# blindopen/TSM-Det-Pointcloud-

Measured on AMD Instinct MI355X. Metric: point-cloud frames/sec (fwd+bwd), higher is better.
Workload: dtype f32; 1 GPU; BASELINE configs[1]: KITTI-shaped synthetic, 20000 pts / 16000 active voxels per frame, full SECOND detector (VoxelBackBone8x) fwd+bwd+AdamW step; batch_per_gpu=4, global_batch=4, parallelism=dp1, voxelize_on_gpu=True

## Files before the change

tsm-det-pointcloud-_amd/csrc/conv_wgrad.hip:

```cpp
#include "spx_common.h"

#ifdef SPX_WG_DIAG
__device__ unsigned long long* g_wg_diag = nullptr;
extern "C" int spx_diag_set(unsigned long long* p) { return (int)hipMemcpyToSymbol(HIP_SYMBOL(g_wg_diag), &p, sizeof(p)); }
#define DIAG_T() __builtin_amdgcn_s_memtime()
#endif

namespace {

typedef float f32x4 __attribute__((ext_vector_type(4)));

#ifndef SPX_SB
#define SPX_SB __builtin_amdgcn_sched_barrier(0)
#endif
constexpr int kGroups = 4;
#ifndef SPX_WG_BURST
#define SPX_WG_BURST 4
#endif
constexpr int kBurst = SPX_WG_BURST;

static inline int wgrad_splits(int64_t n, int cin, int cout, int kvol) {
  int64_t s = n / (64 * kGroups);
  constexpr int slab_mb = 32;
  int64_t by_slab = (int64_t(slab_mb) << 20) / ((int64_t)kvol * cin * cout * 4);
  if (s > by_slab) s = by_slab;
  constexpr int max_blocks = 2048;
  int64_t by_blocks = max_blocks / kvol;
  if (by_blocks < 8) by_blocks = 8;
  if (s > by_blocks) s = by_blocks;
  if (s < 1) s = 1;
  return (int)s;
}

__device__ __forceinline__ void wgrad_plan(const int32_t* __restrict__ cnt, int K, int J, int lane, int& sk, int& start,
                                           int& mycnt) {
  const uint32_t cval = lane < K ? (uint32_t)cnt[lane] : 0u;
  mycnt = (int)cval;
  uint64_t total = cval;
#pragma unroll
  for (int o = 32; o > 0; o >>= 1) total += __shfl_xor(total, o);
  int sh = 0;
  while ((total >> sh) >= (1u << 19)) ++sh;
  const uint32_t tot_s = (uint32_t)(total >> sh);
  sk = 0;
  if (lane < K) sk = tot_s > 0 ? 1 + (int)(((uint32_t)(J - K) * (cval >> sh)) / tot_s) : J / K;
  int incl = sk;
#pragma unroll
  for (int o = 1; o < 64; o <<= 1) {
    int t = __shfl_up(incl, o);
    if (lane >= o) incl += t;
  }
  start = incl - sk;
}

constexpr int kCntUnroll = 4;
__global__ __launch_bounds__(1024) void k_wgrad_count(const int32_t* __restrict__ pair, int64_t ld, int64_t n,
                                                      const int64_t* d_n, int K, int G, int32_t* __restrict__ cnt64,
                                                      int32_t* __restrict__ cnt8) {
  __shared__ int32_t part[16];
  const int x = blockIdx.x, k = blockIdx.y;
  const int lane = threadIdx.x & 63, w = threadIdx.x >> 6;
  const int64_t nlive = spx_live_n(d_n, n);
  const int64_t n8 = ((nlive + 7) / 8 + 63) / 64 * 64;
  const int64_t g0 = x * (n8 / 64);
  int64_t g1 = g0 + n8 / 64;
  const int64_t glive = (nlive + 63) / 64;
  if (g1 > glive) g1 = glive;
  const int32_t* prow = pair + (int64_t)k * ld;
  int total = 0;
  for (int64_t g = g0 + w * kCntUnroll; g < g1; g += 16 * kCntUnroll) {
    int32_t id[kCntUnroll];
#pragma unroll
    for (int u = 0; u < kCntUnroll; ++u) {
      const int64_t row = 64 * (g + u) + lane;
      id[u] = (g + u < g1 && row < nlive) ? prow[row] : -1;
    }
#pragma unroll
    for (int u = 0; u < kCntUnroll; ++u) {
      const int c = __popcll(__ballot(id[u] >= 0));
      if (lane == 0 && g + u < g1) cnt64[(size_t)k * G + g + u] = c;
      total += c;
    }
  }
  if (lane == 0) part[w] = total;
  __syncthreads();
  if (threadIdx.x == 0) {
    int t = 0;
#pragma unroll
    for (int i = 0; i < 16; ++i) t += part[i];
    cnt8[x * 32 + k] = t;
  }
}

template <int W>
__device__ __forceinline__ void load_vec(const float* __restrict__ p, float (&v)[W]) {
  if constexpr (W == 1) {
    v[0] = p[0];
  } else if constexpr (W == 2) {
    float2 t = *reinterpret_cast<const float2*>(p);
    v[0] = t.x, v[1] = t.y;
  } else {
#pragma unroll
    for (int i = 0; i < W; i += 4) {
      float4 t = *reinterpret_cast<const float4*>(p + i);
      v[i] = t.x, v[i + 1] = t.y, v[i + 2] = t.z, v[i + 3] = t.w;
    }
  }
}

template <int W>
__device__ __forceinline__ void store_vec(float* __restrict__ p, const float (&v)[W]) {
  if constexpr (W == 1) {
    p[0] = v[0];
  } else if constexpr (W == 2) {
    *reinterpret_cast<float2*>(p) = make_float2(v[0], v[1]);
  } else {
#pragma unroll
    for (int i = 0; i < W; i += 4) *reinterpret_cast<float4*>(p + i) = make_float4(v[i], v[i + 1], v[i + 2], v[i + 3]);
  }
}

template <int MI, int NJ, bool EXACT, bool FULL>
__device__ __forceinline__ void wgrad_fetch(const float* __restrict__ in, int cin, const float* __restrict__ dout,
                                            int cout, const int32_t* q_src, const int32_t* q_dst, int p, int npairs,
                                            int c, float (&a)[MI], float (&b)[NJ]) {
  const bool has = FULL || (p < npairs);
  const int32_t sid = has ? q_src[p] : 0;
  const int32_t did = has ? q_dst[p] : 0;
  if (EXACT && FULL) {
    load_vec<MI>(in + (size_t)sid * cin + MI * c, a);
    load_vec<NJ>(dout + (size_t)did * cout + NJ * c, b);
  } else {
#pragma unroll
    for (int mi = 0; mi < MI; ++mi) {
      int ci = MI * c + mi;
      a[mi] = (has && ci < cin) ? in[(size_t)sid * cin + ci] : 0.f;
    }
#pragma unroll
    for (int nj = 0; nj < NJ; ++nj) {
      int co = NJ * c + nj;
      b[nj] = (has && co < cout) ? dout[(size_t)did * cout + co] : 0.f;
    }
  }
}

template <int MI, int NJ>
__device__ __forceinline__ void wgrad_mfma_step(f32x4 (&acc)[MI][NJ], const float (&a)[MI], const float (&b)[NJ]) {
#pragma unroll
  for (int mi = 0; mi < MI; ++mi)
#pragma unroll
    for (int nj = 0; nj < NJ; ++nj) acc[mi][nj] = __builtin_amdgcn_mfma_f32_16x16x4f32(a[mi], b[nj], acc[mi][nj], 0, 0, 0);
}

template <int MI, int NJ, bool EXACT>
__global__ __launch_bounds__(64) void k_wgrad_mfma(const float* __restrict__ in, int cin,
                                                   const float* __restrict__ dout, int cout,
                                                   const int32_t* __restrict__ pair, int64_t ld, int64_t n,
                                                   const int64_t* d_n, const int32_t* __restrict__ cnt64,
                                                   const int32_t* __restrict__ cnt8, int G, int J, int K,
                                                   float* __restrict__ slab) {
  __shared__ int32_t q_src[64 * kGroups + 4];
  __shared__ int32_t q_dst[64 * kGroups + 4];
  const int lane = threadIdx.x;
  const int c = lane & 15, q = lane >> 4;
  const int xcd = blockIdx.x & 7, j = blockIdx.x >> 3;
  int sk, start, mycnt;
  wgrad_plan(cnt8 + xcd * 32, K, J, lane, sk, start, mycnt);
  const unsigned long long mine = __ballot(lane < K && j >= start && j < start + sk);
  if (mine == 0) return;
  const int k = __ffsll((long long)mine) - 1;
  const int sub = __builtin_amdgcn_readfirstlane(j - __shfl(start, k));
  const int nsub = __builtin_amdgcn_readfirstlane(__shfl(sk, k));
  const int64_t total = __builtin_amdgcn_readfirstlane(__shfl(mycnt, k));
  const int64_t nlive = spx_live_n(d_n, n);
  const int64_t n8 = ((nlive + 7) / 8 + 63) / 64 * 64;
  const int64_t lo = total * sub / nsub, hi = total * (sub + 1) / nsub;
  const int gx0 = (int)(xcd * (n8 / 64));
  int gx1 = gx0 + (int)(n8 / 64);
  const int glive = (int)((nlive + 63) / 64);
  if (gx1 > glive) gx1 = glive;
  int n_lo = 0, n_hi = 0;
  int64_t run = 0;
  for (int g = gx0; g < gx1; g += 64) {
    const int v = g + lane < gx1 ? cnt64[(size_t)k * G + g + lane] : 0;
    int incl = v;
#pragma unroll
    for (int o = 1; o < 64; o <<= 1) {
      int t = __shfl_up(incl, o);
      if (lane >= o) incl += t;
    }
    const int64_t excl = run + incl - v;
    const bool in = g + lane < gx1;
    n_lo += __popcll(__ballot(in && excl < lo));
    n_hi += __popcll(__ballot(in && excl < hi));
    run += __shfl(incl, 63);
  }
  int64_t r0 = 64 * (int64_t)(gx0 + n_lo);
  int64_t r1 = 64 * (int64_t)(gx0 + n_hi);
  if (r1 > nlive) r1 = nlive;
  if (r0 > r1) r0 = r1;

#ifdef SPX_WG_DIAG
  const unsigned long long d_t0 = DIAG_T(), d_r0 = __builtin_amdgcn_s_memrealtime();
  unsigned long long d_steps = 0, d_loop = 0, d_nsteps = 0;
#endif
  f32x4 acc[MI][NJ];
#pragma unroll
  for (int mi = 0; mi < MI; ++mi)
#pragma unroll
    for (int nj = 0; nj < NJ; ++nj) acc[mi][nj] = f32x4{0.f, 0.f, 0.f, 0.f};

  const int32_t* prow = pair + (int64_t)k * ld;
  int carry = 0;
  int32_t idn[kGroups];
  const int64_t rlast = r1 > r0 ? r1 - 1 : 0;
#pragma unroll
  for (int g = 0; g < kGroups; ++g) {
    int64_t row = r0 + 64 * g + lane;
    idn[g] = prow[row < rlast ? row : rlast];
  }
  for (int64_t base = r0; base < r1; base += 64 * kGroups) {
    int32_t id[kGroups];
#pragma unroll
    for (int g = 0; g < kGroups; ++g) {
      id[g] = base + 64 * g + lane < r1 ? idn[g] : -1;
      int64_t row = base + 64 * (kGroups + g) + lane;
      idn[g] = prow[row < rlast ? row : rlast];
    }
    int nvalid = carry;
#pragma unroll
    for (int g = 0; g < kGroups; ++g) {
      unsigned long long mask = __ballot(id[g] >= 0);
      int rank = nvalid + __builtin_amdgcn_mbcnt_hi((unsigned)(mask >> 32), __builtin_amdgcn_mbcnt_lo((unsigned)mask, 0u));
      if (id[g] >= 0) {
        q_src[rank] = id[g];
        q_dst[rank] = (int32_t)(base + 64 * g + lane);
      }
      nvalid += __popcll(mask);
    }
    const int full = nvalid >> 2;
    carry = nvalid & 3;
    if (full == 0) continue;
    __builtin_amdgcn_wave_barrier();
    const int last = full - 1;
#ifdef SPX_WG_DIAG
    const unsigned long long d_a = DIAG_T();
    d_nsteps += full;
#endif
    for (int st = 0; st < full; st += kBurst) {
      float a[kBurst][MI], b[kBurst][NJ];
#pragma unroll
      for (int g = 0; g < kBurst; ++g) {
        const int sg = st + g < last ? st + g : last;
        wgrad_fetch<MI, NJ, EXACT, true>(in, cin, dout, cout, q_src, q_dst, 4 * sg + q, 4, c, a[g], b[g]);
      }
      asm volatile("" ::: "memory");
      __builtin_amdgcn_sched_barrier(0);
#pragma unroll
      for (int g = 0; g < kBurst; ++g) {
        if (g > 0) {
          const float keep = st + g < full ? 1.f : 0.f;
#pragma unroll
          for (int nj = 0; nj < NJ; ++nj) b[g][nj] *= keep;
        }
        wgrad_mfma_step<MI, NJ>(acc, a[g], b[g]);
      }
    }
#ifdef SPX_WG_DIAG
    d_loop += DIAG_T() - d_a;
#endif
    __builtin_amdgcn_wave_barrier();
    if (carry) {
      int32_t ts = 0, td = 0;
      if (lane < carry) ts = q_src[4 * full + lane], td = q_dst[4 * full + lane];
      __builtin_amdgcn_wave_barrier();
      if (lane < carry) q_src[lane] = ts, q_dst[lane] = td;
    }
    __builtin_amdgcn_wave_barrier();
  }
  int ntail = carry ? 1 : 0;
  ntail = __builtin_amdgcn_readfirstlane(ntail);
  asm volatile("" : "+s"(ntail));
  for (int t = 0; t < ntail; ++t) {
    __builtin_amdgcn_wave_barrier();
    float a0[MI], b0[NJ];
    wgrad_fetch<MI, NJ, EXACT, false>(in, cin, dout, cout, q_src, q_dst, q, carry, c, a0, b0);
    wgrad_mfma_step<MI, NJ>(acc, a0, b0);
  }

#ifdef SPX_WG_DIAG
  if (g_wg_diag && lane == 0) {
    unsigned long long* o = g_wg_diag + (size_t)blockIdx.x * 8;
    const unsigned long long t1 = DIAG_T();
    o[0] = t1 - d_t0;
    o[1] = d_loop;
    o[2] = d_nsteps;
    o[3] = __builtin_amdgcn_s_memrealtime() - d_r0;
    o[4] = k;
    o[5] = d_t0;
    o[6] = t1;
    o[7] = (unsigned long long)(r1 > r0 ? r1 - r0 : 0);
  }
#endif
  float* out = slab + ((size_t)xcd * J + j) * cin * cout;
#pragma unroll
  for (int mi = 0; mi < MI; ++mi)
#pragma unroll
    for (int e = 0; e < 4; ++e) {
      const int ci = MI * (4 * q + e) + mi;
      if (EXACT) {
        float v[NJ];
#pragma unroll
        for (int nj = 0; nj < NJ; ++nj) v[nj] = acc[mi][nj][e];
        store_vec<NJ>(out + (size_t)ci * cout + NJ * c, v);
      } else if (ci < cin) {
#pragma unroll
        for (int nj = 0; nj < NJ; ++nj) {
          int co = NJ * c + nj;
          if (co < cout) out[(size_t)ci * cout + co] = acc[mi][nj][e];
        }
      }
    }
}

constexpr int kRedSlices = 16;
__global__ __launch_bounds__(64 * kRedSlices) void k_wgrad_reduce(const float* __restrict__ slab,
                                                                   const int32_t* __restrict__ cnt8, int J, int K, int cin,
                                                                   int cout, float* __restrict__ dw) {
  __shared__ float part[kRedSlices][64];
  __shared__ int p_off[9][32], p_start[8][32];
  {
    const int w = threadIdx.x >> 6, lane = threadIdx.x & 63;
    if (w < 8) {
      int sk, start, mycnt;
      wgrad_plan(cnt8 + w * 32, K, J, lane, sk, start, mycnt);
      if (lane < 32) p_off[w + 1][lane] = sk, p_start[w][lane] = start;
    }
  }
  __syncthreads();
  if (threadIdx.x < 32) {
    int run = 0;
    for (int x = 0; x < 8; ++x) {
      int v = p_off[x + 1][threadIdx.x];
      p_off[x][threadIdx.x] = run;
      run += v;
    }
    p_off[8][threadIdx.x] = run;
  }
  __syncthreads();
  const int per = cin * cout;
  const int total = K * per;
  const int e = threadIdx.x & 63, sl = threadIdx.x >> 6;
  const int t = blockIdx.x * 64 + e;
  float acc4[4] = {0.f, 0.f, 0.f, 0.f};
  if (t < total) {
    const int k = t / per, el = t - k * per;
    const int len = p_off[8][k];
    int x = 0;
    for (int i = sl; i < len; i += 4 * kRedSlices) {
#pragma unroll
      for (int u = 0; u < 4; ++u) {
        const int ii = i + u * kRedSlices;
        if (ii < len) {
          while (ii >= p_off[x + 1][k]) ++x;
          acc4[u] += slab[((size_t)x * J + p_start[x][k] + (ii - p_off[x][k])) * per + el];
        }
      }
    }
  }
  part[sl][e] = (acc4[0] + acc4[1]) + (acc4[2] + acc4[3]);
  __syncthreads();
  if (sl == 0 && t < total) {
    float v = 0.f;
#pragma unroll
    for (int i = 0; i < kRedSlices; ++i) v += part[i][e];
    int co = t % cout, ci = (t / cout) % cin, k = t / per;
    dw[((size_t)co * K + k) * cin + ci] = v;
  }
}

}

static inline int wgrad_blocks_per_xcd(int64_t n, int cin, int cout, int kvol) {
  int J = (wgrad_splits(n, cin, cout, kvol) * kvol + 7) / 8;
  return J < kvol ? kvol : J;
}

static inline size_t wgrad_slab_bytes(int cin, int cout, int kvol, int64_t n) {
  return spx_align((size_t)8 * wgrad_blocks_per_xcd(n, cin, cout, kvol) * cin * cout * sizeof(float));
}
static inline size_t wgrad_cnt64_bytes(int kvol, int64_t n) {
  return spx_align((size_t)kvol * (size_t)((n + 63) / 64 + 1) * sizeof(int32_t));
}

extern "C" size_t spx_conv_wgrad_ws_bytes(int cin, int cout, int kvol, int64_t n_out) {
  return wgrad_slab_bytes(cin, cout, kvol, n_out) + wgrad_cnt64_bytes(kvol, n_out) + spx_align(8 * 32 * sizeof(int32_t));
}

#define SPX_WG_CASE(A, B)                                                                                          \
  if (MI == A && NJ == B) {                                                                                        \
    if (exact)                                                                                                     \
      hipLaunchKernelGGL((k_wgrad_mfma<A, B, true>), dim3(8 * J), dim3(64), 0, s, in, cin, dout, cout, pair, pair_ld, n_out, \
                         d_n_out, cnt64, cnt8, G, J, kvol, slab);                                                  \
    else                                                                                                           \
      hipLaunchKernelGGL((k_wgrad_mfma<A, B, false>), dim3(8 * J), dim3(64), 0, s, in, cin, dout, cout, pair, pair_ld, n_out, \
                         d_n_out, cnt64, cnt8, G, J, kvol, slab);                                                  \
    launched = true;                                                                                               \
  }

extern "C" size_t spx_conv_wgrad_counts_bytes(int kvol, int64_t n_out) {
  return wgrad_cnt64_bytes(kvol, n_out < 0 ? 0 : n_out) + spx_align(8 * 32 * sizeof(int32_t));
}

extern "C" int spx_conv_wgrad_counts(const int32_t* pair, int64_t pair_ld, int kvol, int64_t n_out, const int64_t* d_n_out,
                                     int32_t* counts, spx_stream_t stream) {
  if (!pair || !counts || kvol <= 0 || kvol > SPX_MAX_KVOL || n_out <= 0 || pair_ld < n_out) return SPX_ERR_INVALID_ARG;
  if (n_out >= (int64_t(1) << 31)) return SPX_ERR_TOO_LARGE;
  const int G = (int)((n_out + 63) / 64 + 1);
  int32_t* cnt8 = reinterpret_cast<int32_t*>(reinterpret_cast<char*>(counts) + wgrad_cnt64_bytes(kvol, n_out));
  hipLaunchKernelGGL(k_wgrad_count, dim3(8, kvol), dim3(1024), 0, spx_s(stream), pair, pair_ld, n_out, d_n_out, kvol, G,
                     counts, cnt8);
  SPX_CHECK_LAUNCH();
  return SPX_OK;
}

extern "C" int spx_conv_wgrad(const float* in, int cin, const float* dout, int cout, int kvol, const int32_t* pair,
                              int64_t pair_ld, int64_t n_out, const int64_t* d_n_out, const int32_t* counts, float* dw,
                              void* ws, size_t ws_bytes, spx_stream_t stream) {
  if (!in || !dout || !pair || !dw || cin <= 0 || cout <= 0 || kvol <= 0 || kvol > SPX_MAX_KVOL || n_out < 0 ||
      pair_ld < n_out)
    return SPX_ERR_INVALID_ARG;
  if (cin > 128 || cout > 128) return SPX_ERR_UNSUPPORTED;
  if (n_out >= (int64_t(1) << 31)) return SPX_ERR_TOO_LARGE;
  if (!ws || ws_bytes < spx_conv_wgrad_ws_bytes(cin, cout, kvol, n_out)) return SPX_ERR_WORKSPACE;
  hipStream_t s = spx_s(stream);
  if (n_out == 0) {
    spx_fill_async(dw, 0, sizeof(float) * (size_t)cout * kvol * cin, s);
    return SPX_OK;
  }
  const int J = wgrad_blocks_per_xcd(n_out, cin, cout, kvol);
  const int G = (int)((n_out + 63) / 64 + 1);
  const int32_t* cnt64 = counts;
  const int32_t* cnt8 = counts ? reinterpret_cast<const int32_t*>(reinterpret_cast<const char*>(counts) + wgrad_cnt64_bytes(kvol, n_out))
                               : nullptr;
  if (!counts) {
    int32_t* c64 = reinterpret_cast<int32_t*>(reinterpret_cast<char*>(ws) + wgrad_slab_bytes(cin, cout, kvol, n_out));
    int32_t* c8 = reinterpret_cast<int32_t*>(reinterpret_cast<char*>(c64) + wgrad_cnt64_bytes(kvol, n_out));
    hipLaunchKernelGGL(k_wgrad_count, dim3(8, kvol), dim3(1024), 0, s, pair, pair_ld, n_out, d_n_out, kvol, G, c64, c8);
    cnt64 = c64;
    cnt8 = c8;
  }
  float* slab = reinterpret_cast<float*>(ws);
  int MI = (cin + 15) / 16, NJ = (cout + 15) / 16;
  if (MI == 3) MI = 4;
  if (MI > 4) MI = 8;
  if (NJ == 3) NJ = 4;
  if (NJ > 4) NJ = 8;
  bool launched = false;
  const bool exact = cin == 16 * MI && cout == 16 * NJ;
  SPX_WG_CASE(1, 1)
  SPX_WG_CASE(1, 2)
  SPX_WG_CASE(1, 4)
  SPX_WG_CASE(1, 8)
  SPX_WG_CASE(2, 1)
  SPX_WG_CASE(2, 2)
  SPX_WG_CASE(2, 4)
  SPX_WG_CASE(2, 8)
  SPX_WG_CASE(4, 1)
  SPX_WG_CASE(4, 2)
  SPX_WG_CASE(4, 4)
  SPX_WG_CASE(4, 8)
  SPX_WG_CASE(8, 1)
  SPX_WG_CASE(8, 2)
  SPX_WG_CASE(8, 4)
  SPX_WG_CASE(8, 8)
  if (!launched) return SPX_ERR_UNSUPPORTED;
  int total = kvol * cin * cout;
  hipLaunchKernelGGL(k_wgrad_reduce, dim3((total + 63) / 64), dim3(64 * kRedSlices), 0, s, slab, cnt8, J, kvol, cin, cout, dw);
  SPX_CHECK_LAUNCH();
  return SPX_OK;
}
```

Baseline: 293.2 frames/s.

## Batch wgrad queue fills, double-buffer gather bursts, and restructure slab reduction

After: 291.5 frames/s. No clear change (-0.6%).

```diff
diff --git a/tsm-det-pointcloud-_amd/csrc/conv_wgrad.hip b/tsm-det-pointcloud-_amd/csrc/conv_wgrad.hip
--- a/tsm-det-pointcloud-_amd/csrc/conv_wgrad.hip
+++ b/tsm-det-pointcloud-_amd/csrc/conv_wgrad.hip
@@ -18,6 +18,12 @@
 #define SPX_WG_BURST 4
 #endif
 constexpr int kBurst = SPX_WG_BURST;
+#ifndef SPX_WG_FILL
+#define SPX_WG_FILL 128
+#endif
+constexpr int kFill = SPX_WG_FILL;
+static_assert(kFill >= 2 * 4 * kBurst, "the fill threshold is at least two bursts");
+constexpr int kQueue = kFill + 64 * kGroups + 4;
 
 static inline int wgrad_splits(int64_t n, int cin, int cout, int kvol) {
   int64_t s = n / (64 * kGroups);
@@ -153,14 +159,47 @@
 }
 
 template <int MI, int NJ, bool EXACT>
+__host__ __device__ constexpr bool wgrad_two_sets() {
+  return EXACT || MI * NJ <= 4;
+}
+
+template <int MI, int NJ, bool EXACT>
+__device__ __forceinline__ void wgrad_fetch_burst(const float* __restrict__ in, int cin, const float* __restrict__ dout,
+                                                  int cout, const int32_t* q_src, const int32_t* q_dst, int st, int last,
+                                                  int q, int c, float (&a)[kBurst][MI], float (&b)[kBurst][NJ]) {
+#pragma unroll
+  for (int g = 0; g < kBurst; ++g) {
+    const int sg = st + g < last ? st + g : last;
+    wgrad_fetch<MI, NJ, EXACT, true>(in, cin, dout, cout, q_src, q_dst, 4 * sg + q, 4, c, a[g], b[g]);
+  }
+  asm volatile("" ::: "memory");
+  __builtin_amdgcn_sched_barrier(0);
+}
+
+template <int MI, int NJ>
+__device__ __forceinline__ void wgrad_mfma_burst(f32x4 (&acc)[MI][NJ], float (&a)[kBurst][MI], float (&b)[kBurst][NJ], int st,
+                                                 int full) {
+#pragma unroll
+  for (int g = 0; g < kBurst; ++g) {
+    if (g > 0) {
+      const float keep = st + g < full ? 1.f : 0.f;
+#pragma unroll
+      for (int nj = 0; nj < NJ; ++nj) b[g][nj] *= keep;
+    }
+    wgrad_mfma_step<MI, NJ>(acc, a[g], b[g]);
+  }
+  __builtin_amdgcn_sched_barrier(0);
+}
+
+template <int MI, int NJ, bool EXACT>
 __global__ __launch_bounds__(64) void k_wgrad_mfma(const float* __restrict__ in, int cin,
                                                    const float* __restrict__ dout, int cout,
                                                    const int32_t* __restrict__ pair, int64_t ld, int64_t n,
                                                    const int64_t* d_n, const int32_t* __restrict__ cnt64,
                                                    const int32_t* __restrict__ cnt8, int G, int J, int K,
                                                    float* __restrict__ slab) {
-  __shared__ int32_t q_src[64 * kGroups + 4];
-  __shared__ int32_t q_dst[64 * kGroups + 4];
+  __shared__ int32_t q_src[kQueue];
+  __shared__ int32_t q_dst[kQueue];
   const int lane = threadIdx.x;
   const int c = lane & 15, q = lane >> 4;
   const int xcd = blockIdx.x & 7, j = blockIdx.x >> 3;
@@ -211,7 +250,7 @@
     for (int nj = 0; nj < NJ; ++nj) acc[mi][nj] = f32x4{0.f, 0.f, 0.f, 0.f};
 
   const int32_t* prow = pair + (int64_t)k * ld;
-  int carry = 0;
+  int nq = 0;
   int32_t idn[kGroups];
   const int64_t rlast = r1 > r0 ? r1 - 1 : 0;
 #pragma unroll
@@ -227,43 +266,45 @@
       int64_t row = base + 64 * (kGroups + g) + lane;
       idn[g] = prow[row < rlast ? row : rlast];
     }
-    int nvalid = carry;
 #pragma unroll
     for (int g = 0; g < kGroups; ++g) {
       unsigned long long mask = __ballot(id[g] >= 0);
-      int rank = nvalid + __builtin_amdgcn_mbcnt_hi((unsigned)(mask >> 32), __builtin_amdgcn_mbcnt_lo((unsigned)mask, 0u));
+      int rank = nq + __builtin_amdgcn_mbcnt_hi((unsigned)(mask >> 32), __builtin_amdgcn_mbcnt_lo((unsigned)mask, 0u));
       if (id[g] >= 0) {
         q_src[rank] = id[g];
         q_dst[rank] = (int32_t)(base + 64 * g + lane);
       }
-      nvalid += __popcll(mask);
-    }
-    const int full = nvalid >> 2;
-    carry = nvalid & 3;
+      nq += __popcll(mask);
+    }
+    if (nq < kFill && base + 64 * kGroups < r1) continue;
+    const int full = nq >> 2;
     if (full == 0) continue;
+    const int carry = nq & 3;
     __builtin_amdgcn_wave_barrier();
     const int last = full - 1;
 #ifdef SPX_WG_DIAG
     const unsigned long long d_a = DIAG_T();
     d_nsteps += full;
 #endif
-    for (int st = 0; st < full; st += kBurst) {
-      float a[kBurst][MI], b[kBurst][NJ];
-#pragma unroll
-      for (int g = 0; g < kBurst; ++g) {
-        const int sg = st + g < last ? st + g : last;
-        wgrad_fetch<MI, NJ, EXACT, true>(in, cin, dout, cout, q_src, q_dst, 4 * sg + q, 4, c, a[g], b[g]);
+    if constexpr (wgrad_two_sets<MI, NJ, EXACT>()) {
+      float a0[kBurst][MI], b0[kBurst][NJ], a1[kBurst][MI], b1[kBurst][NJ];
+      const int nburst = (full + kBurst - 1) / kBurst;
+      wgrad_fetch_burst<MI, NJ, EXACT>(in, cin, dout, cout, q_src, q_dst, 0, last, q, c, a0, b0);
+      int st = 0;
+      for (int i = 0; i < (nburst >> 1); ++i, st += 2 * kBurst) {
+        wgrad_fetch_burst<MI, NJ, EXACT>(in, cin, dout, cout, q_src, q_dst, st + kBurst, last, q, c, a1, b1);
+        wgrad_mfma_burst<MI, NJ>(acc, a0, b0, st, full);
+        wgrad_fetch_burst<MI, NJ, EXACT>(in, cin, dout, cout, q_src, q_dst, st + 2 * kBurst, last, q, c, a0, b0);
+        wgrad_mfma_burst<MI, NJ>(acc, a1, b1, st + kBurst, full);
       }
-      asm volatile("" ::: "memory");
-      __builtin_amdgcn_sched_barrier(0);
-#pragma unroll
-      for (int g = 0; g < kBurst; ++g) {
-        if (g > 0) {
-          const float keep = st + g < full ? 1.f : 0.f;
-#pragma unroll
-          for (int nj = 0; nj < NJ; ++nj) b[g][nj] *= keep;
-        }
-        wgrad_mfma_step<MI, NJ>(acc, a[g], b[g]);
+      int nodd = __builtin_amdgcn_readfirstlane(nburst & 1);
+      asm volatile("" : "+s"(nodd));
+      if (nodd) wgrad_mfma_burst<MI, NJ>(acc, a0, b0, st, full);
+    } else {
+      for (int st = 0; st < full; st += kBurst) {
+        float a[kBurst][MI], b[kBurst][NJ];
+        wgrad_fetch_burst<MI, NJ, EXACT>(in, cin, dout, cout, q_src, q_dst, st, last, q, c, a, b);
+        wgrad_mfma_burst<MI, NJ>(acc, a, b, st, full);
       }
     }
 #ifdef SPX_WG_DIAG
@@ -276,8 +317,10 @@
       __builtin_amdgcn_wave_barrier();
       if (lane < carry) q_src[lane] = ts, q_dst[lane] = td;
     }
+    nq = carry;
     __builtin_amdgcn_wave_barrier();
   }
+  const int carry = nq;
   int ntail = carry ? 1 : 0;
   ntail = __builtin_amdgcn_readfirstlane(ntail);
   asm volatile("" : "+s"(ntail));
@@ -324,58 +367,72 @@
 }
 
 constexpr int kRedSlices = 16;
-__global__ __launch_bounds__(64 * kRedSlices) void k_wgrad_reduce(const float* __restrict__ slab,
-                                                                   const int32_t* __restrict__ cnt8, int J, int K, int cin,
-                                                                   int cout, float* __restrict__ dw) {
-  __shared__ float part[kRedSlices][64];
-  __shared__ int p_off[9][32], p_start[8][32];
-  {
-    const int w = threadIdx.x >> 6, lane = threadIdx.x & 63;
-    if (w < 8) {
-      int sk, start, mycnt;
-      wgrad_plan(cnt8 + w * 32, K, J, lane, sk, start, mycnt);
-      if (lane < 32) p_off[w + 1][lane] = sk, p_start[w][lane] = start;
-    }
+constexpr int kRedThreads = 256;
+constexpr int kRedMaxSlots = 8 * 256;
+__global__ __launch_bounds__(kRedThreads) void k_wgrad_reduce(const float* __restrict__ slab,
+                                                              const int32_t* __restrict__ cnt8, int J, int K, int cin,
+                                                              int cout, int passes, float* __restrict__ dw) {
+  __shared__ float part[2][kRedSlices][64];
+  __shared__ int s_sk[8], s_start[8];
+  __shared__ int s_slot[kRedMaxSlots];
+  const int k = blockIdx.y;
+  const int w = __builtin_amdgcn_readfirstlane(threadIdx.x >> 6), lane = threadIdx.x & 63;
+#pragma unroll
+  for (int x = w; x < 8; x += kRedThreads / 64) {
+    int sk, start, mycnt;
+    wgrad_plan(cnt8 + x * 32, K, J, lane, sk, start, mycnt);
+    if (lane == k) s_sk[x] = sk, s_start[x] = start;
   }
   __syncthreads();
-  if (threadIdx.x < 32) {
-    int run = 0;
-    for (int x = 0; x < 8; ++x) {
-      int v = p_off[x + 1][threadIdx.x];
-      p_off[x][threadIdx.x] = run;
-      run += v;
-    }
-    p_off[8][threadIdx.x] = run;
+  int off[9];
+  off[0] = 0;
+#pragma unroll
+  for (int x = 0; x < 8; ++x) off[x + 1] = off[x] + s_sk[x];
+  const int len = off[8];
+  for (int i = threadIdx.x; i < len; i += kRedThreads) {
+    int slot = 0;
+#pragma unroll
+    for (int x = 0; x < 8; ++x)
+      if (i >= off[x] && i < off[x + 1]) slot = x * J + s_start[x] + (i - off[x]);
+    s_slot[i] = slot;
   }
   __syncthreads();
   const int per = cin * cout;
-  const int total = K * per;
-  const int e = threadIdx.x & 63, sl = threadIdx.x >> 6;
-  const int t = blockIdx.x * 64 + e;
-  float acc4[4] = {0.f, 0.f, 0.f, 0.f};
-  if (t < total) {
-    const int k = t / per, el = t - k * per;
-    const int len = p_off[8][k];
-    int x = 0;
-    for (int i = sl; i < len; i += 4 * kRedSlices) {
-#pragma unroll
-      for (int u = 0; u < 4; ++u) {
-        const int ii = i + u * kRedSlices;
-        if (ii < len) {
-          while (ii >= p_off[x + 1][k]) ++x;
-          acc4[u] += slab[((size_t)x * J + p_start[x][k] + (ii - p_off[x][k])) * per + el];
+  for (int p = 0; p < passes; ++p) {
+    const int el0 = (blockIdx.x * passes + p) * 64;
+    if (el0 >= per) break;
+    const int el = el0 + lane;
+    const float* src = slab + (el < per ? el : per - 1);
+    float acc[4][4];
+#pragma unroll
+    for (int s = 0; s < 4; ++s)
+#pragma unroll
+      for (int u = 0; u < 4; ++u) acc[s][u] = 0.f;
+    for (int base = 0; base < len; base += 4 * kRedSlices) {
+      float v[4][4];
+#pragma unroll
+      for (int u = 0; u < 4; ++u)
+#pragma unroll
+        for (int s = 0; s < 4; ++s) {
+          const int i = base + u * kRedSlices + 4 * w + s;
+          v[s][u] = src[(size_t)s_slot[i < len ? i : len - 1] * per];
         }
-      }
-    }
-  }
-  part[sl][e] = (acc4[0] + acc4[1]) + (acc4[2] + acc4[3]);
-  __syncthreads();
-  if (sl == 0 && t < total) {
-    float v = 0.f;
-#pragma unroll
-    for (int i = 0; i < kRedSlices; ++i) v += part[i][e];
-    int co = t % cout, ci = (t / cout) % cin, k = t / per;
-    dw[((size_t)co * K + k) * cin + ci] = v;
+#pragma unroll
+      for (int u = 0; u < 4; ++u)
+#pragma unroll
+        for (int s = 0; s < 4; ++s)
+          if (base + u * kRedSlices + 4 * w + s < len) acc[s][u] += v[s][u];
+    }
+#pragma unroll
+    for (int s = 0; s < 4; ++s) part[p & 1][4 * w + s][lane] = (acc[s][0] + acc[s][1]) + (acc[s][2] + acc[s][3]);
+    __syncthreads();
+    if (w == 0 && el < per) {
+      float r = 0.f;
+#pragma unroll
+      for (int i = 0; i < kRedSlices; ++i) r += part[p & 1][i][lane];
+      const int co = el % cout, ci = el / cout;
+      dw[((size_t)co * K + k) * cin + ci] = r;
+    }
   }
 }
 
@@ -440,6 +497,7 @@
   }
   const int J = wgrad_blocks_per_xcd(n_out, cin, cout, kvol);
   const int G = (int)((n_out + 63) / 64 + 1);
+  if (8 * J > kRedMaxSlots) return SPX_ERR_UNSUPPORTED;
   const int32_t* cnt64 = counts;
   const int32_t* cnt8 = counts ? reinterpret_cast<const int32_t*>(reinterpret_cast<const char*>(counts) + wgrad_cnt64_bytes(kvol, n_out))
                                : nullptr;
@@ -475,8 +533,11 @@
   SPX_WG_CASE(8, 4)
   SPX_WG_CASE(8, 8)
   if (!launched) return SPX_ERR_UNSUPPORTED;
-  int total = kvol * cin * cout;
-  hipLaunchKernelGGL(k_wgrad_reduce, dim3((total + 63) / 64), dim3(64 * kRedSlices), 0, s, slab, cnt8, J, kvol, cin, cout, dw);
+  constexpr int kRedBlocks = 1024;
+  const int strips = (cin * cout + 63) / 64;
+  const int passes = (kvol * strips + kRedBlocks - 1) / kRedBlocks;
+  hipLaunchKernelGGL(k_wgrad_reduce, dim3((strips + passes - 1) / passes, kvol), dim3(kRedThreads), 0, s, slab, cnt8, J,
+                     kvol, cin, cout, passes, dw);
   SPX_CHECK_LAUNCH();
   return SPX_OK;
 }
```
